# taconite/IntrinsicAvatar

Hardware: AMD Instinct MI355X
Metric: rays/sec (fwd+bwd) at 540×540, 1024 spp; fraction of HBM / MFMA roofline (higher is better)
Workload: dtype f32

## Files before the change

intrinsicavatar_amd/csrc/hashgrid.hip:

```cpp
#include <stdlib.h>

#include "ia_common.h"

namespace {

constexpr int THREADS = 256;
constexpr int MAX_LEVELS = 32;

struct HashCfg {
    int n_levels;
    uint32_t offsets[MAX_LEVELS + 1];
    uint32_t res[MAX_LEVELS];
    float scale[MAX_LEVELS];
};

__host__ void make_cfg(HashCfg& c, int n_levels, int log2_hashmap_size, int base_resolution, float per_level_scale)
{
    c.n_levels = n_levels;
    uint32_t offset = 0;
    const float l2 = log2f(per_level_scale);
    for (int l = 0; l < n_levels; l++) {
        const float sc = exp2f((float)l * l2) * (float)base_resolution - 1.0f;
        const uint32_t res = (uint32_t)ceilf(sc) + 1u;
        const uint32_t max_params = 0xFFFFFFFFu / 2;
        uint32_t p = powf((float)res, 3.0f) > (float)max_params ? max_params : res * res * res;
        p = (p + 7u) / 8u * 8u;
        const uint32_t cap = 1u << log2_hashmap_size;
        if (p > cap) p = cap;
        c.offsets[l] = offset;
        c.res[l] = res;
        c.scale[l] = sc;
        offset += p;
    }
    c.offsets[n_levels] = offset;
}

__device__ __forceinline__ uint32_t grid_index(uint32_t hsize, uint32_t res, uint32_t px, uint32_t py, uint32_t pz)
{
    uint32_t stride = 1, index = 0;
    bool hashed = false;
    index += px * stride; stride *= res;
    if (stride <= hsize) { index += py * stride; stride *= res; } else hashed = true;
    if (!hashed && stride <= hsize) { index += pz * stride; stride *= res; } else hashed = true;
    if (hsize < stride) index = (px * 1u) ^ (py * 2654435761u) ^ (pz * 805459861u);
    return ((hsize & (hsize - 1u)) == 0u) ? (index & (hsize - 1u)) : (index % hsize);
}

typedef float f4_a8 __attribute__((ext_vector_type(4), aligned(8)));

template <bool WITH_JAC>
__global__ __launch_bounds__(THREADS) __attribute__((amdgpu_waves_per_eu(4, 4))) void hash_fwd_kernel(int64_t n, const float* __restrict__ x,
                                                            const float2* __restrict__ params, HashCfg cfg,
                                                            float* __restrict__ out, int out_stride,
                                                            float* __restrict__ dy_dx)
{
    const int L = cfg.n_levels;
    const int64_t t = (int64_t)blockIdx.x * THREADS + threadIdx.x;
    const int64_t i = t / L;
    const int l = (int)(t % L);
    if (i >= n) return;
    const float sc = cfg.scale[l];
    const uint32_t res = cfg.res[l], hsize = cfg.offsets[l + 1] - cfg.offsets[l];
    const float2* tab = params + cfg.offsets[l];
    float pos[3];
    uint32_t pg[3];
#pragma unroll
    for (int d = 0; d < 3; d++) {
        const float p = fmaf(sc, x[i * 3 + d], 0.5f);
        const float fl = floorf(p);
        pg[d] = (uint32_t)(int)fl;
        pos[d] = p - fl;
    }
    float2 v[8];
#pragma unroll
    for (int c = 0; c < 8; c++) {
        const uint32_t idx = grid_index(hsize, res, pg[0] + (c & 1), pg[1] + ((c >> 1) & 1), pg[2] + ((c >> 2) & 1));
        v[c] = tab[idx];
    }
    float a0 = 0.f, a1 = 0.f;
    float j0[3] = {0.f, 0.f, 0.f}, j1[3] = {0.f, 0.f, 0.f};
#pragma unroll
    for (int c = 0; c < 8; c++) {
        const float wx = (c & 1) ? pos[0] : 1.0f - pos[0];
        const float wy = (c & 2) ? pos[1] : 1.0f - pos[1];
        const float wz = (c & 4) ? pos[2] : 1.0f - pos[2];
        const float w = wx * wy * wz;
        a0 = fmaf(w, v[c].x, a0);
        a1 = fmaf(w, v[c].y, a1);
        if (WITH_JAC) {
            const float dx = ((c & 1) ? sc : -sc) * wy * wz;
            const float dy = ((c & 2) ? sc : -sc) * wx * wz;
            const float dz = ((c & 4) ? sc : -sc) * wx * wy;
            j0[0] = fmaf(dx, v[c].x, j0[0]); j0[1] = fmaf(dy, v[c].x, j0[1]); j0[2] = fmaf(dz, v[c].x, j0[2]);
            j1[0] = fmaf(dx, v[c].y, j1[0]); j1[1] = fmaf(dy, v[c].y, j1[1]); j1[2] = fmaf(dz, v[c].y, j1[2]);
        }
    }
    *reinterpret_cast<float2*>(out + i * out_stride + l * 2) = make_float2(a0, a1);
    if (WITH_JAC) {
        float* J = dy_dx + (i * L * 2 + l * 2) * 3;
        J[0] = j0[0]; J[1] = j0[1]; J[2] = j0[2];
        J[3] = j1[0]; J[4] = j1[1]; J[5] = j1[2];
    }
}


struct XcdPlan {
    int first_level[8], n_level[8];
    int part[8], nparts[8];
    int straight;
};

typedef float f4_a8b __attribute__((ext_vector_type(4), aligned(8)));
__device__ __forceinline__ void load_x_pair(const float2* __restrict__ tab, uint32_t i0, uint32_t i1, float2& v0, float2& v1)
{
    if (i1 == i0 + 1u) {
        const f4_a8b q = *reinterpret_cast<const f4_a8b*>(tab + i0);
        v0 = make_float2(q.x, q.y); v1 = make_float2(q.z, q.w);
    } else if (i0 == i1 + 1u) {
        const f4_a8b q = *reinterpret_cast<const f4_a8b*>(tab + i1);
        v1 = make_float2(q.x, q.y); v0 = make_float2(q.z, q.w);
    } else {
        v0 = tab[i0];
        v1 = tab[i1];
    }
}
template <bool WITH_JAC>
__device__ __forceinline__ void xcd_gather(const float2* __restrict__ tab, uint32_t hsize, uint32_t res, float sc,
                                           const float xs[3], float2 v[8], float pos[3])
{
    uint32_t pg[3];
#pragma unroll
    for (int d = 0; d < 3; d++) {
        const float p = fmaf(sc, xs[d], 0.5f);
        const float fl = floorf(p);
        pg[d] = (uint32_t)(int)fl;
        pos[d] = p - fl;
    }
#pragma unroll
    for (int c = 0; c < 8; c += 2) {
        const uint32_t i0 = grid_index(hsize, res, pg[0], pg[1] + ((c >> 1) & 1), pg[2] + ((c >> 2) & 1));
        const uint32_t i1 = grid_index(hsize, res, pg[0] + 1u, pg[1] + ((c >> 1) & 1), pg[2] + ((c >> 2) & 1));
        load_x_pair(tab, i0, i1, v[c], v[c + 1]);
    }
}

template <bool HASHED>
__device__ __forceinline__ uint32_t level_index(uint32_t hsize, uint32_t res, uint32_t px, uint32_t py, uint32_t pz)
{
    if (HASHED) return ((px * 1u) ^ (py * 2654435761u) ^ (pz * 805459861u)) & (hsize - 1u);
    const uint32_t index = px + res * (py + res * pz);
    return min(index >= hsize ? index - hsize : index, hsize - 1u);
}

template <bool HASHED>
__device__ __forceinline__ void xcd_gather2(const float2* __restrict__ tab, uint32_t hsize, uint32_t res, float sc, const float xa[3],
                                            const float xb[3], float2 va[8], float2 vb[8], float pa[3], float pb[3])
{
    typedef float v2f __attribute__((ext_vector_type(2)));
    typedef float f4_a16 __attribute__((ext_vector_type(4), aligned(16)));
    uint32_t ga[3], gb[3];
#pragma unroll
    for (int d = 0; d < 3; d++) {
        const float p = fmaf(sc, xa[d], 0.5f), fl = floorf(p);
        ga[d] = (uint32_t)(int)fl; pa[d] = p - fl;
        const float p2 = fmaf(sc, xb[d], 0.5f), fl2 = floorf(p2);
        gb[d] = (uint32_t)(int)fl2; pb[d] = p2 - fl2;
    }
    uint32_t i0[8], i1[8];
#pragma unroll
    for (int c = 0; c < 4; c++) {
        i0[c] = level_index<HASHED>(hsize, res, ga[0], ga[1] + (c & 1), ga[2] + ((c >> 1) & 1));
        i1[c] = level_index<HASHED>(hsize, res, ga[0] + 1u, ga[1] + (c & 1), ga[2] + ((c >> 1) & 1));
        i0[4 + c] = level_index<HASHED>(hsize, res, gb[0], gb[1] + (c & 1), gb[2] + ((c >> 1) & 1));
        i1[4 + c] = level_index<HASHED>(hsize, res, gb[0] + 1u, gb[1] + (c & 1), gb[2] + ((c >> 1) & 1));
    }
    f4_a16 q[8];
    v2f t[8];
#pragma unroll
    for (int c = 0; c < 8; c++) {
        q[c] = *reinterpret_cast<const f4_a16*>(tab + (i0[c] & ~1u));
        t[c] = *reinterpret_cast<const v2f*>(tab + i1[c]);
    }
#pragma unroll
    for (int c = 0; c < 8; c++) {
        const bool odd = (i0[c] & 1u) != 0u;
        const float2 lo = make_float2(q[c].x, q[c].y), hi = make_float2(q[c].z, q[c].w);
        const float2 e0 = odd ? hi : lo;
        const float2 e1 = (i1[c] == (i0[c] ^ 1u)) ? (odd ? lo : hi) : make_float2(t[c].x, t[c].y);
        if (c < 4) { va[2 * c] = e0; va[2 * c + 1] = e1; } else { vb[2 * (c - 4)] = e0; vb[2 * (c - 4) + 1] = e1; }
    }
    if (!HASHED) {
        if (ga[0] > res || ga[1] > res || ga[2] > res)
#pragma unroll
            for (int c = 0; c < 8; c++) va[c] = tab[grid_index(hsize, res, ga[0] + (c & 1), ga[1] + ((c >> 1) & 1), ga[2] + ((c >> 2) & 1))];
        if (gb[0] > res || gb[1] > res || gb[2] > res)
#pragma unroll
            for (int c = 0; c < 8; c++) vb[c] = tab[grid_index(hsize, res, gb[0] + (c & 1), gb[1] + ((c >> 1) & 1), gb[2] + ((c >> 2) & 1))];
    }
}

template <bool WITH_JAC>
__device__ __forceinline__ void xcd_blend_store(const float2 v[8], const float pos[3], float sc, int64_t slot,
                                                float2* __restrict__ tmp, float* __restrict__ tmp_jac)
{
    float a0 = 0.f, a1 = 0.f;
    float j0[3] = {0.f, 0.f, 0.f}, j1[3] = {0.f, 0.f, 0.f};
#pragma unroll
    for (int c = 0; c < 8; c++) {
        const float wx = (c & 1) ? pos[0] : 1.0f - pos[0];
        const float wy = (c & 2) ? pos[1] : 1.0f - pos[1];
        const float wz = (c & 4) ? pos[2] : 1.0f - pos[2];
        const float w = wx * wy * wz;
        a0 = fmaf(w, v[c].x, a0);
        a1 = fmaf(w, v[c].y, a1);
        if (WITH_JAC) {
            const float dx = ((c & 1) ? sc : -sc) * wy * wz;
            const float dy = ((c & 2) ? sc : -sc) * wx * wz;
            const float dz = ((c & 4) ? sc : -sc) * wx * wy;
            j0[0] = fmaf(dx, v[c].x, j0[0]); j0[1] = fmaf(dy, v[c].x, j0[1]); j0[2] = fmaf(dz, v[c].x, j0[2]);
            j1[0] = fmaf(dx, v[c].y, j1[0]); j1[1] = fmaf(dy, v[c].y, j1[1]); j1[2] = fmaf(dz, v[c].y, j1[2]);
        }
    }
    typedef float v2f __attribute__((ext_vector_type(2)));
    __builtin_nontemporal_store((v2f){a0, a1}, reinterpret_cast<v2f*>(tmp + slot));
    if (WITH_JAC) {
        v2f* J = reinterpret_cast<v2f*>(tmp_jac + slot * 6);
        __builtin_nontemporal_store((v2f){j0[0], j0[1]}, J);
        __builtin_nontemporal_store((v2f){j0[2], j1[0]}, J + 1);
        __builtin_nontemporal_store((v2f){j1[1], j1[2]}, J + 2);
    }
}

template <bool WITH_JAC>
__global__ __launch_bounds__(THREADS) void hash_fwd_xcd_kernel(int64_t n, const float* __restrict__ x,
                                                                const float2* __restrict__ params, HashCfg cfg, XcdPlan plan,
                                                                float2* __restrict__ tmp ,
                                                                float* __restrict__ tmp_jac )
{
    const int slot = blockIdx.x & 7;
    const int64_t chunk = blockIdx.x >> 3, nchunks = gridDim.x >> 3;
    const int np = plan.nparts[slot];
    const int64_t per = (n + np - 1) / np;
    const int64_t lo = per * plan.part[slot], hi = (lo + per < n) ? lo + per : n;
    const int64_t stride = nchunks * THREADS;
    for (int64_t i = lo + chunk * THREADS + threadIdx.x; i < hi; i += 2 * stride) {
        const int64_t i2 = i + stride;
        const bool two = i2 < hi;
        const int64_t ib = two ? i2 : i;
        const float xa[3] = {__builtin_nontemporal_load(x + i * 3 + 0), __builtin_nontemporal_load(x + i * 3 + 1),
                             __builtin_nontemporal_load(x + i * 3 + 2)};
        const float xb[3] = {__builtin_nontemporal_load(x + ib * 3 + 0), __builtin_nontemporal_load(x + ib * 3 + 1),
                             __builtin_nontemporal_load(x + ib * 3 + 2)};
        for (int l = plan.first_level[slot]; l < plan.first_level[slot] + plan.n_level[slot]; l++) {
            const float sc = cfg.scale[l];
            const uint32_t res = cfg.res[l], hsize = cfg.offsets[l + 1] - cfg.offsets[l];
            const float2* tab = params + cfg.offsets[l];
            float2 va[8], vb[8];
            float pa[3], pb[3];
            const uint64_t r64 = res;
            const bool hashed = r64 * r64 * r64 > (uint64_t)hsize;
            if (plan.straight && hashed && (hsize & (hsize - 1u)) == 0u) xcd_gather2<true>(tab, hsize, res, sc, xa, xb, va, vb, pa, pb);
            else if (plan.straight && !hashed) xcd_gather2<false>(tab, hsize, res, sc, xa, xb, va, vb, pa, pb);
            else {
                xcd_gather<WITH_JAC>(tab, hsize, res, sc, xa, va, pa);
                xcd_gather<WITH_JAC>(tab, hsize, res, sc, xb, vb, pb);
            }
            xcd_blend_store<WITH_JAC>(va, pa, sc, (int64_t)l * n + i, tmp, tmp_jac);
            if (two) xcd_blend_store<WITH_JAC>(vb, pb, sc, (int64_t)l * n + i2, tmp, tmp_jac);
        }
    }
}

template <bool WITH_JAC>
__global__ __launch_bounds__(THREADS) void hash_transpose_kernel(int64_t n, int L, const float2* __restrict__ tmp,
                                                                  const float* __restrict__ tmp_jac, float* __restrict__ out,
                                                                  int out_stride, float* __restrict__ dy_dx)
{
    extern __shared__ __attribute__((aligned(16))) float s_t[];
    const int64_t p0 = (int64_t)blockIdx.x * THREADS;
    const int rows = (int)((n - p0) < THREADS ? (n - p0) : THREADS);
    const int ld = 2 * L + 1;
    for (int l = 0; l < L; l++)
        if ((int)threadIdx.x < rows) {
            const float2 v = tmp[(int64_t)l * n + p0 + threadIdx.x];
            s_t[threadIdx.x * ld + 2 * l] = v.x; s_t[threadIdx.x * ld + 2 * l + 1] = v.y;
        }
    __syncthreads();
    for (int i = threadIdx.x; i < rows * 2 * L; i += THREADS) {
        const int r = i / (2 * L), c = i % (2 * L);
        out[(p0 + r) * out_stride + c] = s_t[r * ld + c];
    }
    if (WITH_JAC) {
        __syncthreads();
        const int ldj = 6 * L + 1;
        for (int l = 0; l < L; l++)
            if ((int)threadIdx.x < rows) {
                const float* J = tmp_jac + ((int64_t)l * n + p0 + threadIdx.x) * 6;
#pragma unroll
                for (int k = 0; k < 6; k++) s_t[threadIdx.x * ldj + 6 * l + k] = J[k];
            }
        __syncthreads();
        for (int i = threadIdx.x; i < rows * 6 * L; i += THREADS) {
            const int r = i / (6 * L), c = i % (6 * L);
            dy_dx[(p0 + r) * 6 * L + c] = s_t[r * ldj + c];
        }
    }
}

template <bool SECOND>
__global__ __launch_bounds__(THREADS) void hash_bwd_runs_kernel(int64_t n, const float* __restrict__ x, HashCfg cfg,
                                                                 const float* __restrict__ gE, int gE_stride,
                                                                 const float* __restrict__ gG, int gG_stride,
                                                                 const float* __restrict__ q, float* __restrict__ grad)
{
    const int64_t i = (int64_t)blockIdx.x * THREADS + threadIdx.x;
    const int lane = threadIdx.x & 63;
    const bool active = i < n;
    const int64_t ii = active ? i : n - 1;
    const float x0 = x[ii * 3 + 0], x1 = x[ii * 3 + 1], x2 = x[ii * 3 + 2];
    float qx = 0.f, qy = 0.f, qz = 0.f;
    if (SECOND) { qx = q[ii * 3 + 0]; qy = q[ii * 3 + 1]; qz = q[ii * 3 + 2]; }
    for (int l = 0; l < cfg.n_levels; l++) {
        const float sc = cfg.scale[l];
        const uint32_t res = cfg.res[l], hsize = cfg.offsets[l + 1] - cfg.offsets[l];
        float* tab = grad + (int64_t)cfg.offsets[l] * 2;
        float2 e = make_float2(0.f, 0.f), g = make_float2(0.f, 0.f);
        if (active) {
            if (gE) e = *reinterpret_cast<const float2*>(gE + i * gE_stride + l * 2);
            if (SECOND) g = *reinterpret_cast<const float2*>(gG + i * gG_stride + l * 2);
        }
        const bool any_here = (e.x != 0.f) || (e.y != 0.f) || (g.x != 0.f) || (g.y != 0.f);
        if (!__any(any_here)) continue;
        float pos[3];
        uint32_t pg[3];
        {
            const float xs[3] = {x0, x1, x2};
#pragma unroll
            for (int d = 0; d < 3; d++) {
                const float p = fmaf(sc, xs[d], 0.5f);
                const float fl = floorf(p);
                pg[d] = (uint32_t)(int)fl;
                pos[d] = p - fl;
            }
        }
#pragma unroll
        for (int c = 0; c < 8; c++) {
            const float wx = (c & 1) ? pos[0] : 1.0f - pos[0];
            const float wy = (c & 2) ? pos[1] : 1.0f - pos[1];
            const float wz = (c & 4) ? pos[2] : 1.0f - pos[2];
            const float w0 = wx * wy * wz;
            float vx = e.x * w0, vy = e.y * w0;
            if (SECOND) {
                const float dw = ((c & 1) ? sc : -sc) * wy * wz * qx + ((c & 2) ? sc : -sc) * wx * wz * qy +
                                 ((c & 4) ? sc : -sc) * wx * wy * qz;
                vx += g.x * dw;
                vy += g.y * dw;
            }
            uint32_t idx = grid_index(hsize, res, pg[0] + (c & 1), pg[1] + ((c >> 1) & 1), pg[2] + ((c >> 2) & 1));
            if (!active) { idx = 0xFFFFFFFFu; vx = 0.f; vy = 0.f; }
            const uint32_t prev = __shfl_up(idx, 1, 64);
            const bool head = (lane == 0) || (prev != idx);
            const unsigned long long heads = __ballot(head);
            const unsigned long long below = heads & ((lane == 63) ? ~0ull : ((1ull << (lane + 1)) - 1ull));
            const int hpos = 63 - __clzll(below);
#pragma unroll
            for (int off = 1; off < 64; off <<= 1) {
                const float ax = __shfl_up(vx, off, 64), ay = __shfl_up(vy, off, 64);
                if (lane - off >= hpos) { vx += ax; vy += ay; }
            }
            const bool tail = (lane == 63) || ((heads >> (lane + 1)) & 1ull);
            if (tail && active && (vx != 0.f || vy != 0.f)) {
                unsafeAtomicAdd(tab + (int64_t)idx * 2 + 0, vx);
                unsafeAtomicAdd(tab + (int64_t)idx * 2 + 1, vy);
            }
        }
    }
}


constexpr int SLICE_LOG2 = 13;
constexpr int SLICE = 1 << SLICE_LOG2;
constexpr int BIN_ROUNDS = 4;
constexpr int BIN_TILE = THREADS * BIN_ROUNDS;
constexpr int MAX_BUCKETS = 1024;
constexpr int MAX_PARTS = 64;
constexpr int PART_RECORDS = 1 << 19;

struct BinCfg {
    int n_buckets;
    int bstart[MAX_LEVELS + 1];
};

__host__ void make_bins(BinCfg& b, const HashCfg& c)
{
    int k = 0;
    for (int l = 0; l < c.n_levels; l++) {
        b.bstart[l] = k;
        k += (int)((c.offsets[l + 1] - c.offsets[l] + SLICE - 1) >> SLICE_LOG2);
    }
    b.bstart[c.n_levels] = k;
    b.n_buckets = k;
}

__device__ __forceinline__ void level_max_update(unsigned* p, float lmax)
{
    const unsigned v = __float_as_uint(lmax);
    if (v > __atomic_load_n(p, __ATOMIC_RELAXED)) atomicMax(p, v);
}

template <bool SECOND, bool FILL>
__global__ __launch_bounds__(THREADS) void hash_bin_kernel(int64_t n, const float* __restrict__ x, HashCfg cfg, BinCfg bins,
                                                            const float* __restrict__ gE, int gE_stride,
                                                            const float* __restrict__ gG, int gG_stride,
                                                            const float* __restrict__ q, int nwg,
                                                            int32_t* __restrict__ counts, uint16_t* __restrict__ rec_idx,
                                                            float2* __restrict__ rec_val, uint32_t level_mask,
                                                            unsigned* __restrict__ level_max)
{
    __shared__ int hist[MAX_BUCKETS];
    __shared__ int base[FILL ? MAX_BUCKETS : 1];
    const int lane = threadIdx.x & 63;
// ... 433 lines not shown
}

__global__ __launch_bounds__(THREADS) void sh4_bwd_kernel(int64_t n, const float* __restrict__ d01,
                                                           const float* __restrict__ g, int g_stride,
                                                           float* __restrict__ g_d01)
{
    const int64_t i = (int64_t)blockIdx.x * THREADS + threadIdx.x;
    if (i >= n) return;
    const float x = d01[i * 3 + 0] * 2.f - 1.f, y = d01[i * 3 + 1] * 2.f - 1.f, z = d01[i * 3 + 2] * 2.f - 1.f;
    const float x2 = x * x, y2 = y * y, z2 = z * z;
    const float* go = g + i * g_stride;
    float gx = 0.f, gy = 0.f, gz = 0.f;
    gy += go[1] * -0.48860251190291987f;
    gz += go[2] * 0.48860251190291987f;
    gx += go[3] * -0.48860251190291987f;
    gx += go[4] * 1.0925484305920792f * y;           gy += go[4] * 1.0925484305920792f * x;
    gy += go[5] * -1.0925484305920792f * z;          gz += go[5] * -1.0925484305920792f * y;
    gz += go[6] * 2.0f * 0.94617469575755997f * z;
    gx += go[7] * -1.0925484305920792f * z;          gz += go[7] * -1.0925484305920792f * x;
    gx += go[8] * 2.0f * 0.54627421529603959f * x;   gy += go[8] * -2.0f * 0.54627421529603959f * y;
    gx += go[9] * 0.59004358992664352f * y * (-6.0f * x);
    gy += go[9] * 0.59004358992664352f * (-3.0f * x2 + 3.0f * y2);
    gx += go[10] * 2.8906114426405538f * y * z;      gy += go[10] * 2.8906114426405538f * x * z;
    gz += go[10] * 2.8906114426405538f * x * y;
    gy += go[11] * 0.45704579946446572f * (1.0f - 5.0f * z2);
    gz += go[11] * 0.45704579946446572f * y * (-10.0f * z);
    gz += go[12] * 0.3731763325901154f * (15.0f * z2 - 3.0f);
    gx += go[13] * 0.45704579946446572f * (1.0f - 5.0f * z2);
    gz += go[13] * 0.45704579946446572f * x * (-10.0f * z);
    gx += go[14] * 1.4453057213202769f * z * 2.0f * x; gy += go[14] * 1.4453057213202769f * z * -2.0f * y;
    gz += go[14] * 1.4453057213202769f * (x2 - y2);
    gx += go[15] * 0.59004358992664352f * (-3.0f * x2 + 3.0f * y2);
    gy += go[15] * 0.59004358992664352f * x * 6.0f * y;
    g_d01[i * 3 + 0] = 2.0f * gx; g_d01[i * 3 + 1] = 2.0f * gy; g_d01[i * 3 + 2] = 2.0f * gz;
}

template <int MODE>
__global__ __launch_bounds__(THREADS) void jac_contract_kernel(int64_t n, int K, const float* __restrict__ jac,
                                                                const float* __restrict__ v, int v_stride,
                                                                float* __restrict__ out, int out_stride)
{
    if (MODE == 0) {
        const int64_t i = (int64_t)blockIdx.x * THREADS + threadIdx.x;
        if (i >= n) return;
        float a0 = 0.f, a1 = 0.f, a2 = 0.f;
        const float* J = jac + i * K * 3;
        for (int k = 0; k < K; k++) {
            const float g = v[i * v_stride + k];
            a0 = fmaf(g, J[k * 3 + 0], a0); a1 = fmaf(g, J[k * 3 + 1], a1); a2 = fmaf(g, J[k * 3 + 2], a2);
        }
        out[i * out_stride + 0] = a0; out[i * out_stride + 1] = a1; out[i * out_stride + 2] = a2;
    } else {
        const int64_t t = (int64_t)blockIdx.x * THREADS + threadIdx.x;
        const int64_t i = t / K;
        const int k = (int)(t % K);
        if (i >= n) return;
        const float* J = jac + (i * K + k) * 3;
        out[i * out_stride + k] = J[0] * v[i * v_stride + 0] + J[1] * v[i * v_stride + 1] + J[2] * v[i * v_stride + 2];
    }
}

}

IA_EXPORT int ia_hashgrid_jac_contract(int mode, int64_t n, int K, const float* jac, const float* v, int v_stride,
                                       float* out, int out_stride, ia_stream_t stream)
{
    if (n == 0) return IA_OK;
    IA_REQUIRE(mode == 0 || mode == 1, "mode 0 (J^T v) or 1 (J q)");
    if (mode == 0)
        jac_contract_kernel<0><<<ia::cdiv(n, THREADS), THREADS, 0, (hipStream_t)stream>>>(n, K, jac, v, v_stride, out, out_stride);
    else
        jac_contract_kernel<1><<<ia::cdiv(n * K, THREADS), THREADS, 0, (hipStream_t)stream>>>(n, K, jac, v, v_stride, out, out_stride);
    return ia::check_launch("ia_hashgrid_jac_contract");
}

IA_EXPORT int ia_sh4_bwd(int64_t n, const float* d01, const float* g_sh, int g_stride, float* g_d01, ia_stream_t stream)
{
    if (n == 0) return IA_OK;
    sh4_bwd_kernel<<<ia::cdiv(n, THREADS), THREADS, 0, (hipStream_t)stream>>>(n, d01, g_sh, g_stride, g_d01);
    return ia::check_launch("ia_sh4_bwd");
}

IA_EXPORT int64_t ia_hashgrid_n_entries(int n_levels, int log2_hashmap_size, int base_resolution, float per_level_scale)
{
    if (n_levels <= 0 || n_levels > MAX_LEVELS) return -1;
    HashCfg c;
    make_cfg(c, n_levels, log2_hashmap_size, base_resolution, per_level_scale);
    return (int64_t)c.offsets[n_levels];
}

IA_EXPORT int ia_hashgrid_fwd(int64_t n, const float* x, const float* params, int n_levels, int n_features,
                              int log2_hashmap_size, int base_resolution, float per_level_scale, float* out,
                              int out_stride, float* dy_dx, ia_stream_t stream)
{
    if (n == 0) return IA_OK;
    IA_REQUIRE(n_features == 2, "n_features_per_level must be 2 on this path");
    IA_REQUIRE(n_levels > 0 && n_levels <= MAX_LEVELS, "n_levels out of range");
    IA_REQUIRE(out_stride >= n_levels * 2 && (out_stride % 2) == 0, "out_stride must be even and >= n_levels*2");
    HashCfg c;
    make_cfg(c, n_levels, log2_hashmap_size, base_resolution, per_level_scale);
    const int grid = ia::cdiv(n * n_levels, THREADS);
    hipStream_t s = (hipStream_t)stream;
    if (dy_dx) hash_fwd_kernel<true><<<grid, THREADS, 0, s>>>(n, x, (const float2*)params, c, out, out_stride, dy_dx);
    else hash_fwd_kernel<false><<<grid, THREADS, 0, s>>>(n, x, (const float2*)params, c, out, out_stride, nullptr);
    return ia::check_launch("ia_hashgrid_fwd");
}


struct HashFwdScratch {
    float2* feat;
    float* jac;
    int64_t jac_offset;
};

static size_t hash_fwd_layout(void* scratch, int64_t n, int n_levels, int with_jac, HashFwdScratch* o)
{
    ia::Carver c(nullptr);
    c.take<float2>((size_t)(n * n_levels), 1);
    c.align_to(256);
    o->jac_offset = (int64_t)c.used();
    if (with_jac) c.take<float>((size_t)(n * n_levels) * 6, 1);
    c.skip(256);
    o->feat = reinterpret_cast<float2*>(scratch);
    o->jac = scratch && with_jac ? reinterpret_cast<float*>(reinterpret_cast<char*>(scratch) + o->jac_offset) : nullptr;
    return c.used();
}

IA_EXPORT int64_t ia_hashgrid_fwd_scratch_bytes(int64_t n, int n_levels, int with_jac)
{
    if (n < 0 || n_levels <= 0 || n_levels > MAX_LEVELS) return -1;
    HashFwdScratch w;
    return (int64_t)hash_fwd_layout(nullptr, n, n_levels, with_jac, &w);
}

IA_EXPORT int ia_hashgrid_fwd_xcd(int64_t n, const float* x, const float* params, int n_levels, int n_features,
                                  int log2_hashmap_size, int base_resolution, float per_level_scale, float* out,
                                  int out_stride, float* dy_dx, void* scratch, ia_stream_t stream)
{
    if (n == 0) return IA_OK;
    IA_REQUIRE(n_features == 2, "n_features_per_level must be 2 on this path");
    IA_REQUIRE(n_levels > 0 && n_levels <= MAX_LEVELS, "n_levels out of range");
    IA_REQUIRE((reinterpret_cast<uintptr_t>(params) & 15) == 0, "ia_hashgrid_fwd_xcd: the table must be 16-byte aligned (entry pairs are read with one aligned 16-byte load)");
    IA_REQUIRE(scratch != nullptr, "scratch required");
    HashCfg c;
    make_cfg(c, n_levels, log2_hashmap_size, base_resolution, per_level_scale);
    HashFwdScratch w;
    hash_fwd_layout(scratch, n, n_levels, dy_dx != nullptr, &w);
    float2* tmp = w.feat;
    float* tmp_jac = w.jac;
    const uint32_t cap = 1u << log2_hashmap_size;
    int n_small = 0;
    while (n_small < n_levels && c.offsets[n_small + 1] - c.offsets[n_small] < cap) n_small++;
    hipStream_t s = (hipStream_t)stream;
    static int chunks_jac = 0, chunks_plain = 0;
    if (!chunks_plain) {
        int dev = 0, n_cu = 256, b0 = 0, b1 = 0;
        (void)hipGetDevice(&dev);
        (void)hipDeviceGetAttribute(&n_cu, hipDeviceAttributeMultiprocessorCount, dev);
        (void)hipOccupancyMaxActiveBlocksPerMultiprocessor(&b0, hash_fwd_xcd_kernel<false>, THREADS, 0);
        (void)hipOccupancyMaxActiveBlocksPerMultiprocessor(&b1, hash_fwd_xcd_kernel<true>, THREADS, 0);
        (void)hipGetLastError();
        const int per_xcd = n_cu >= 8 ? n_cu / 8 : 1;
        chunks_plain = (b0 > 6 ? 6 : (b0 > 0 ? b0 : 4)) * per_xcd;
        chunks_jac = (b1 > 6 ? 6 : (b1 > 0 ? b1 : 4)) * per_xcd;
        if (const char* e = getenv("IA_HASH_XCD_CHUNKS")) chunks_plain = chunks_jac = atoi(e);
    }
    const int chunks = dy_dx ? chunks_jac : chunks_plain;
    int l = n_small;
    bool small_done = (n_small == 0);
    static const int plan_env = getenv("IA_HASH_XCD_PLAN") ? (getenv("IA_HASH_XCD_PLAN")[0] == 'p' ? 1 : 2) : 0;
    const bool by_level = plan_env == 2 || (plan_env == 0 && n >= 300000);
    static const int lpl = getenv("IA_HASH_LEVELS_PER_LAUNCH") ? max(1, atoi(getenv("IA_HASH_LEVELS_PER_LAUNCH"))) : 1;
    if (by_level) {
        for (int u = (n_small > 0 ? -1 : 0); u < n_levels - n_small; u += (u < 0 ? 1 : lpl)) {
            XcdPlan plan;
            plan.straight = 1;
            for (int k = 0; k < 8; k++) {
                plan.first_level[k] = u < 0 ? 0 : n_small + u;
                plan.n_level[k] = u < 0 ? n_small : min(lpl, n_levels - n_small - u);
                plan.part[k] = k; plan.nparts[k] = 8;
            }
            if (dy_dx) hash_fwd_xcd_kernel<true><<<8 * chunks, THREADS, 0, s>>>(n, x, (const float2*)params, c, plan, tmp, tmp_jac);
            else hash_fwd_xcd_kernel<false><<<8 * chunks, THREADS, 0, s>>>(n, x, (const float2*)params, c, plan, tmp, nullptr);
        }
        l = n_levels;
        small_done = true;
    }
    while (l < n_levels || !small_done) {
        XcdPlan plan;
        plan.straight = 1;
        const int big_left = n_levels - l;
        if (big_left >= 8) {
            for (int k = 0; k < 8; k++) { plan.first_level[k] = l + k; plan.n_level[k] = 1; plan.part[k] = 0; plan.nparts[k] = 1; }
            l += 8;
        } else {
            const int units = big_left + (small_done ? 0 : 1);
            static const float small_cost = getenv("IA_HASH_SMALL_COST") ? (float)atof(getenv("IA_HASH_SMALL_COST")) : 1.0f;
            float w[9];
            int share[9], used = 0;
            for (int u = 0; u < units; u++) { w[u] = (!small_done && u == units - 1) ? small_cost : 1.0f; share[u] = 1; used++; }
            for (; used < 8; used++) {
                int best = 0;
                for (int u = 1; u < units; u++) if (w[u] / share[u] > w[best] / share[best]) best = u;
                share[best]++;
            }
            int k = 0;
            for (int u = 0; u < units; u++) {
                const bool is_small = (!small_done && u == units - 1);
                for (int j = 0; j < share[u]; j++, k++) {
                    plan.first_level[k] = is_small ? 0 : l + u;
                    plan.n_level[k] = is_small ? n_small : 1;
                    plan.part[k] = j; plan.nparts[k] = share[u];
                }
            }
            l = n_levels;
            small_done = true;
        }
        if (dy_dx) hash_fwd_xcd_kernel<true><<<8 * chunks, THREADS, 0, s>>>(n, x, (const float2*)params, c, plan, tmp, tmp_jac);
        else hash_fwd_xcd_kernel<false><<<8 * chunks, THREADS, 0, s>>>(n, x, (const float2*)params, c, plan, tmp, nullptr);
    }
    if (out == nullptr) return ia::check_launch("ia_hashgrid_fwd_xcd");
    const size_t lds = sizeof(float) * THREADS * (dy_dx ? 6 * n_levels + 1 : 2 * n_levels + 1);
    static bool attr = false;
    if (!attr) {
        (void)hipFuncSetAttribute((const void*)hash_transpose_kernel<true>, hipFuncAttributeMaxDynamicSharedMemorySize, 128 * 1024);
        (void)hipGetLastError();
        attr = true;
    }
    if (dy_dx) hash_transpose_kernel<true><<<ia::cdiv(n, THREADS), THREADS, lds, s>>>(n, n_levels, tmp, tmp_jac, out, out_stride, dy_dx);
    else hash_transpose_kernel<false><<<ia::cdiv(n, THREADS), THREADS, lds, s>>>(n, n_levels, tmp, nullptr, out, out_stride, nullptr);
    return ia::check_launch("ia_hashgrid_fwd_xcd");
}

IA_EXPORT int64_t ia_hashgrid_fwd_levels_jac_offset(int64_t n, int n_levels)
{
    HashFwdScratch w;
    hash_fwd_layout(nullptr, n, n_levels, 1, &w);
    return w.jac_offset;
}

IA_EXPORT int ia_hashgrid_fwd_levels(int64_t n, const float* x, const float* params, int n_levels, int n_features, int log2_hashmap_size,
                                     int base_resolution, float per_level_scale, int with_jac, void* scratch, ia_stream_t stream)
{
    return ia_hashgrid_fwd_xcd(n, x, params, n_levels, n_features, log2_hashmap_size, base_resolution, per_level_scale, nullptr, 0,
                               with_jac ? reinterpret_cast<float*>(scratch) : nullptr, scratch, stream);
}

IA_EXPORT int ia_hashgrid_bwd(int64_t n, const float* x, int n_levels, int n_features, int log2_hashmap_size,
                              int base_resolution, float per_level_scale, const float* g_enc, int g_enc_stride,
                              const float* g_jac, int g_jac_stride, const float* q, float* grad_params,
                              ia_stream_t stream)
{
    if (n == 0) return IA_OK;
    IA_REQUIRE(n_features == 2, "n_features_per_level must be 2 on this path");
    IA_REQUIRE(n_levels > 0 && n_levels <= MAX_LEVELS, "n_levels out of range");
    IA_REQUIRE(g_enc != nullptr || g_jac != nullptr, "need g_enc and/or g_jac");
    IA_REQUIRE((g_jac == nullptr) == (q == nullptr), "g_jac and q go together");
    HashCfg c;
    make_cfg(c, n_levels, log2_hashmap_size, base_resolution, per_level_scale);
    hipStream_t s = (hipStream_t)stream;
    const int grid = ia::cdiv(n, THREADS);
    if (g_jac) hash_bwd_runs_kernel<true><<<grid, THREADS, 0, s>>>(n, x, c, g_enc, g_enc_stride, g_jac, g_jac_stride, q, grad_params);
    else hash_bwd_runs_kernel<false><<<grid, THREADS, 0, s>>>(n, x, c, g_enc, g_enc_stride, nullptr, 0, nullptr, grad_params);
    return ia::check_launch("ia_hashgrid_bwd");
}


namespace {
struct BinLayout {
    int nwg; int64_t m, records;
    int32_t *counts, *total;
    unsigned* level_max;
    int32_t* plan;
    void* tmp;
    float2* rec_val;
    uint16_t* rec_idx;
    bool fits;
};
bool staged_fill()
{
    static int mode = -1;
    if (mode < 0) {
        const char* e = getenv("IA_HASHBWD_FILL");
        mode = (e && e[0] == 'd') ? 0 : 1;
    }
    return mode == 1;
}

size_t bin_layout(void* scratch, size_t bytes, int64_t n, int n_levels, int n_buckets, BinLayout* L)
{
    L->nwg = staged_fill() ? ia::cdiv(n, U_PTS) : ia::cdiv(n, BIN_TILE);
    L->m = (int64_t)n_buckets * L->nwg;
    L->records = n * n_levels * 8;
    ia::Carver c(scratch, bytes);
    L->counts = c.take<int32_t>((size_t)L->m);
    L->total = c.take<int32_t>(1);
    L->level_max = c.take<unsigned>(MAX_LEVELS);
    L->plan = c.take<int32_t>(MAX_BUCKETS + 64);
    L->tmp = c.take<char>((size_t)ia_scan_tmp_bytes(L->m));
    L->rec_val = c.take<float2>((size_t)L->records);
    L->rec_idx = c.take<uint16_t>((size_t)L->records);
    L->fits = c.fits();
    return c.need(1);
}
}

IA_EXPORT int64_t ia_hashgrid_bwd_scratch_bytes(int64_t n, int n_levels, int log2_hashmap_size, int base_resolution,
                                                float per_level_scale)
{
    if (n_levels <= 0 || n_levels > MAX_LEVELS || n < 0) return -1;
    HashCfg c;
    make_cfg(c, n_levels, log2_hashmap_size, base_resolution, per_level_scale);
    BinCfg b;
    make_bins(b, c);
    if (b.n_buckets > MAX_BUCKETS) return -1;
    BinLayout L;
    return (int64_t)bin_layout(nullptr, SIZE_MAX, n, n_levels, b.n_buckets, &L);
}

IA_EXPORT int ia_hashgrid_bwd_binned(int64_t n, const float* x, int n_levels, int n_features, int log2_hashmap_size,
                                     int base_resolution, float per_level_scale, const float* g_enc, int g_enc_stride,
                                     const float* g_jac, int g_jac_stride, const float* q, float* grad_params,
                                     uint32_t level_mask, void* scratch, int64_t scratch_bytes, ia_stream_t stream)
{
    if (n == 0) return IA_OK;
    IA_REQUIRE(n_features == 2, "n_features_per_level must be 2 on this path");
    IA_REQUIRE(n_levels > 0 && n_levels <= MAX_LEVELS, "n_levels out of range");
    IA_REQUIRE(g_enc != nullptr || g_jac != nullptr, "need g_enc and/or g_jac");
    IA_REQUIRE((g_jac == nullptr) == (q == nullptr), "g_jac and q go together");
    IA_REQUIRE(n * n_levels * 8 < (int64_t)0x7FFFFFFF, "n too large for 32-bit record offsets: split the batch");
    HashCfg c;
    make_cfg(c, n_levels, log2_hashmap_size, base_resolution, per_level_scale);
    BinCfg b;
    make_bins(b, c);
    IA_REQUIRE(b.n_buckets <= MAX_BUCKETS, "too many (level, slice) buckets");
    BinLayout L;
    bin_layout(scratch, scratch_bytes > 0 ? (size_t)scratch_bytes : 0, n, n_levels, b.n_buckets, &L);
    IA_REQUIRE(scratch != nullptr && L.fits, "scratch smaller than ia_hashgrid_bwd_scratch_bytes(n)");
    int32_t *counts = L.counts, *total = L.total;
    void* tmp = L.tmp;
    float2* rec_val = L.rec_val;
    uint16_t* rec_idx = L.rec_idx;
    hipStream_t s = (hipStream_t)stream;
    unsigned* level_max = L.level_max;
    if (hipMemsetAsync(level_max, 0, MAX_LEVELS * sizeof(unsigned), s) != hipSuccess) return ia::check_launch("ia_hashgrid_bwd_binned(memset)");
    const bool staged = staged_fill();
    const int ugrid = ia::cdiv(L.nwg, U_WAVES);
    constexpr size_t lds_count = (size_t)U_WAVES * MAX_BUCKETS * sizeof(int), lds_fill = (size_t)U_WAVES * sizeof(UnitLds);
    if (staged) {
        if (g_jac) hash_bin_unit_kernel<true, false><<<ugrid, THREADS, lds_count, s>>>(n, x, c, b, g_enc, g_enc_stride, g_jac, g_jac_stride, q, L.nwg, L.m, counts, total, rec_idx, rec_val, level_mask, level_max);
        else hash_bin_unit_kernel<false, false><<<ugrid, THREADS, lds_count, s>>>(n, x, c, b, g_enc, g_enc_stride, nullptr, 0, nullptr, L.nwg, L.m, counts, total, rec_idx, rec_val, level_mask, level_max);
    } else {
        if (g_jac) hash_bin_kernel<true, false><<<L.nwg, THREADS, 0, s>>>(n, x, c, b, g_enc, g_enc_stride, g_jac, g_jac_stride, q, L.nwg, counts, rec_idx, rec_val, level_mask, level_max);
        else hash_bin_kernel<false, false><<<L.nwg, THREADS, 0, s>>>(n, x, c, b, g_enc, g_enc_stride, nullptr, 0, nullptr, L.nwg, counts, rec_idx, rec_val, level_mask, level_max);
    }
    int r = ia_exclusive_scan_i32(counts, counts, total, L.m, tmp, stream);
    if (r != IA_OK) return r;
    static bool attr_fill = false;
    if (staged && !attr_fill) {
        (void)hipFuncSetAttribute((const void*)hash_bin_unit_kernel<true, true>, hipFuncAttributeMaxDynamicSharedMemorySize, (int)lds_fill);
        (void)hipFuncSetAttribute((const void*)hash_bin_unit_kernel<false, true>, hipFuncAttributeMaxDynamicSharedMemorySize, (int)lds_fill);
        (void)hipGetLastError();
        attr_fill = true;
    }
    if (staged) {
        if (g_jac) hash_bin_unit_kernel<true, true><<<ugrid, THREADS, lds_fill, s>>>(n, x, c, b, g_enc, g_enc_stride, g_jac, g_jac_stride, q, L.nwg, L.m, counts, total, rec_idx, rec_val, level_mask, level_max);
        else hash_bin_unit_kernel<false, true><<<ugrid, THREADS, lds_fill, s>>>(n, x, c, b, g_enc, g_enc_stride, nullptr, 0, nullptr, L.nwg, L.m, counts, total, rec_idx, rec_val, level_mask, level_max);
    } else {
        if (g_jac) hash_bin_kernel<true, true><<<L.nwg, THREADS, 0, s>>>(n, x, c, b, g_enc, g_enc_stride, g_jac, g_jac_stride, q, L.nwg, counts, rec_idx, rec_val, level_mask, level_max);
        else hash_bin_kernel<false, true><<<L.nwg, THREADS, 0, s>>>(n, x, c, b, g_enc, g_enc_stride, nullptr, 0, nullptr, L.nwg, counts, rec_idx, rec_val, level_mask, level_max);
    }
    static bool attr = false;
// ... 20 lines not shown
```

Baseline: 1.008 million.

## Generalize hashgrid XCD gather to N points per thread with single-entry loads

The XCD forward kernel now processes a compile-time number of points per thread (4 without Jacobian, 2 with) instead of a fixed two, to put more independent gathers in flight and hide hash-table latency. It also adds a load mode that fetches each corner as a separate 8-byte load instead of a 16-byte pair load plus a fallback, and makes that the default. Occupancy-based chunk sizing is now computed per kernel variant. More points per thread raises register pressure and may lower occupancy.

```diff
diff --git a/intrinsicavatar_amd/csrc/hashgrid.hip b/intrinsicavatar_amd/csrc/hashgrid.hip
--- a/intrinsicavatar_amd/csrc/hashgrid.hip
+++ b/intrinsicavatar_amd/csrc/hashgrid.hip
@@ -1,4 +1,5 @@
 #include <stdlib.h>
+#include <string.h>
 
 #include "ia_common.h"
 
@@ -152,50 +153,70 @@
     return min(index >= hsize ? index - hsize : index, hsize - 1u);
 }
 
-template <bool HASHED>
-__device__ __forceinline__ void xcd_gather2(const float2* __restrict__ tab, uint32_t hsize, uint32_t res, float sc, const float xa[3],
-                                            const float xb[3], float2 va[8], float2 vb[8], float pa[3], float pb[3])
+enum { HASH_LOADS_PAIR = 0, HASH_LOADS_SINGLE = 1 };
+#ifndef IA_HASH_NPTS
+#define IA_HASH_NPTS 4
+#endif
+#ifndef IA_HASH_NPTS_JAC
+#define IA_HASH_NPTS_JAC 2
+#endif
+
+template <bool HASHED, int LOADS, int NPTS>
+__device__ __forceinline__ void xcd_gather2(const float2* __restrict__ tab, uint32_t hsize, uint32_t res, float sc,
+                                            const float (&xs)[NPTS][3], float2 (&v)[NPTS][8], float (&pos)[NPTS][3])
 {
     typedef float v2f __attribute__((ext_vector_type(2)));
     typedef float f4_a16 __attribute__((ext_vector_type(4), aligned(16)));
-    uint32_t ga[3], gb[3];
-#pragma unroll
-    for (int d = 0; d < 3; d++) {
-        const float p = fmaf(sc, xa[d], 0.5f), fl = floorf(p);
-        ga[d] = (uint32_t)(int)fl; pa[d] = p - fl;
-        const float p2 = fmaf(sc, xb[d], 0.5f), fl2 = floorf(p2);
-        gb[d] = (uint32_t)(int)fl2; pb[d] = p2 - fl2;
-    }
-    uint32_t i0[8], i1[8];
-#pragma unroll
-    for (int c = 0; c < 4; c++) {
-        i0[c] = level_index<HASHED>(hsize, res, ga[0], ga[1] + (c & 1), ga[2] + ((c >> 1) & 1));
-        i1[c] = level_index<HASHED>(hsize, res, ga[0] + 1u, ga[1] + (c & 1), ga[2] + ((c >> 1) & 1));
-        i0[4 + c] = level_index<HASHED>(hsize, res, gb[0], gb[1] + (c & 1), gb[2] + ((c >> 1) & 1));
-        i1[4 + c] = level_index<HASHED>(hsize, res, gb[0] + 1u, gb[1] + (c & 1), gb[2] + ((c >> 1) & 1));
-    }
-    f4_a16 q[8];
-    v2f t[8];
-#pragma unroll
-    for (int c = 0; c < 8; c++) {
-        q[c] = *reinterpret_cast<const f4_a16*>(tab + (i0[c] & ~1u));
-        t[c] = *reinterpret_cast<const v2f*>(tab + i1[c]);
-    }
-#pragma unroll
-    for (int c = 0; c < 8; c++) {
-        const bool odd = (i0[c] & 1u) != 0u;
-        const float2 lo = make_float2(q[c].x, q[c].y), hi = make_float2(q[c].z, q[c].w);
-        const float2 e0 = odd ? hi : lo;
-        const float2 e1 = (i1[c] == (i0[c] ^ 1u)) ? (odd ? lo : hi) : make_float2(t[c].x, t[c].y);
-        if (c < 4) { va[2 * c] = e0; va[2 * c + 1] = e1; } else { vb[2 * (c - 4)] = e0; vb[2 * (c - 4) + 1] = e1; }
+    uint32_t g[NPTS][3];
+#pragma unroll
+    for (int d = 0; d < 3; d++)
+#pragma unroll
+        for (int p = 0; p < NPTS; p++) {
+            const float q = fmaf(sc, xs[p][d], 0.5f), fl = floorf(q);
+            g[p][d] = (uint32_t)(int)fl; pos[p][d] = q - fl;
+        }
+    uint32_t i0[4 * NPTS], i1[4 * NPTS];
+#pragma unroll
+    for (int c = 0; c < 4; c++)
+#pragma unroll
+        for (int p = 0; p < NPTS; p++) {
+            i0[4 * p + c] = level_index<HASHED>(hsize, res, g[p][0], g[p][1] + (c & 1), g[p][2] + ((c >> 1) & 1));
+            i1[4 * p + c] = level_index<HASHED>(hsize, res, g[p][0] + 1u, g[p][1] + (c & 1), g[p][2] + ((c >> 1) & 1));
+        }
+    if (LOADS == HASH_LOADS_SINGLE) {
+        v2f e0[4 * NPTS], e1[4 * NPTS];
+#pragma unroll
+        for (int c = 0; c < 4 * NPTS; c++) {
+            e0[c] = *reinterpret_cast<const v2f*>(tab + i0[c]);
+            e1[c] = *reinterpret_cast<const v2f*>(tab + i1[c]);
+        }
+#pragma unroll
+        for (int c = 0; c < 4 * NPTS; c++) {
+            v[c >> 2][2 * (c & 3)] = make_float2(e0[c].x, e0[c].y);
+            v[c >> 2][2 * (c & 3) + 1] = make_float2(e1[c].x, e1[c].y);
+        }
+    } else {
+        f4_a16 q[4 * NPTS];
+        v2f t[4 * NPTS];
+#pragma unroll
+        for (int c = 0; c < 4 * NPTS; c++) {
+            q[c] = *reinterpret_cast<const f4_a16*>(tab + (i0[c] & ~1u));
+            t[c] = *reinterpret_cast<const v2f*>(tab + i1[c]);
+        }
+#pragma unroll
+        for (int c = 0; c < 4 * NPTS; c++) {
+            const bool odd = (i0[c] & 1u) != 0u;
+            const float2 lo = make_float2(q[c].x, q[c].y), hi = make_float2(q[c].z, q[c].w);
+            v[c >> 2][2 * (c & 3)] = odd ? hi : lo;
+            v[c >> 2][2 * (c & 3) + 1] = (i1[c] == (i0[c] ^ 1u)) ? (odd ? lo : hi) : make_float2(t[c].x, t[c].y);
+        }
     }
     if (!HASHED) {
-        if (ga[0] > res || ga[1] > res || ga[2] > res)
-#pragma unroll
-            for (int c = 0; c < 8; c++) va[c] = tab[grid_index(hsize, res, ga[0] + (c & 1), ga[1] + ((c >> 1) & 1), ga[2] + ((c >> 2) & 1))];
-        if (gb[0] > res || gb[1] > res || gb[2] > res)
-#pragma unroll
-            for (int c = 0; c < 8; c++) vb[c] = tab[grid_index(hsize, res, gb[0] + (c & 1), gb[1] + ((c >> 1) & 1), gb[2] + ((c >> 2) & 1))];
+#pragma unroll
+        for (int p = 0; p < NPTS; p++)
+            if (g[p][0] > res || g[p][1] > res || g[p][2] > res)
+#pragma unroll
+                for (int c = 0; c < 8; c++) v[p][c] = tab[grid_index(hsize, res, g[p][0] + (c & 1), g[p][1] + ((c >> 1) & 1), g[p][2] + ((c >> 2) & 1))];
     }
 }
 
@@ -231,7 +252,7 @@
     }
 }
 
-template <bool WITH_JAC>
+template <bool WITH_JAC, int LOADS, int NPTS>
 __global__ __launch_bounds__(THREADS) void hash_fwd_xcd_kernel(int64_t n, const float* __restrict__ x,
                                                                 const float2* __restrict__ params, HashCfg cfg, XcdPlan plan,
                                                                 float2* __restrict__ tmp ,
@@ -243,30 +264,33 @@
     const int64_t per = (n + np - 1) / np;
     const int64_t lo = per * plan.part[slot], hi = (lo + per < n) ? lo + per : n;
     const int64_t stride = nchunks * THREADS;
-    for (int64_t i = lo + chunk * THREADS + threadIdx.x; i < hi; i += 2 * stride) {
-        const int64_t i2 = i + stride;
-        const bool two = i2 < hi;
-        const int64_t ib = two ? i2 : i;
-        const float xa[3] = {__builtin_nontemporal_load(x + i * 3 + 0), __builtin_nontemporal_load(x + i * 3 + 1),
-                             __builtin_nontemporal_load(x + i * 3 + 2)};
-        const float xb[3] = {__builtin_nontemporal_load(x + ib * 3 + 0), __builtin_nontemporal_load(x + ib * 3 + 1),
-                             __builtin_nontemporal_load(x + ib * 3 + 2)};
+    for (int64_t i = lo + chunk * THREADS + threadIdx.x; i < hi; i += NPTS * stride) {
+        bool on[NPTS];
+        float xs[NPTS][3];
+#pragma unroll
+        for (int p = 0; p < NPTS; p++) {
+            on[p] = i + p * stride < hi;
+            const int64_t ip = on[p] ? i + p * stride : i;
+#pragma unroll
+            for (int d = 0; d < 3; d++) xs[p][d] = __builtin_nontemporal_load(x + ip * 3 + d);
+        }
         for (int l = plan.first_level[slot]; l < plan.first_level[slot] + plan.n_level[slot]; l++) {
             const float sc = cfg.scale[l];
             const uint32_t res = cfg.res[l], hsize = cfg.offsets[l + 1] - cfg.offsets[l];
             const float2* tab = params + cfg.offsets[l];
-            float2 va[8], vb[8];
-            float pa[3], pb[3];
+            float2 v[NPTS][8];
+            float pos[NPTS][3];
             const uint64_t r64 = res;
             const bool hashed = r64 * r64 * r64 > (uint64_t)hsize;
-            if (plan.straight && hashed && (hsize & (hsize - 1u)) == 0u) xcd_gather2<true>(tab, hsize, res, sc, xa, xb, va, vb, pa, pb);
-            else if (plan.straight && !hashed) xcd_gather2<false>(tab, hsize, res, sc, xa, xb, va, vb, pa, pb);
+            if (plan.straight && hashed && (hsize & (hsize - 1u)) == 0u) xcd_gather2<true, LOADS, NPTS>(tab, hsize, res, sc, xs, v, pos);
+            else if (plan.straight && !hashed) xcd_gather2<false, LOADS, NPTS>(tab, hsize, res, sc, xs, v, pos);
             else {
-                xcd_gather<WITH_JAC>(tab, hsize, res, sc, xa, va, pa);
-                xcd_gather<WITH_JAC>(tab, hsize, res, sc, xb, vb, pb);
-            }
-            xcd_blend_store<WITH_JAC>(va, pa, sc, (int64_t)l * n + i, tmp, tmp_jac);
-            if (two) xcd_blend_store<WITH_JAC>(vb, pb, sc, (int64_t)l * n + i2, tmp, tmp_jac);
+#pragma unroll
+                for (int p = 0; p < NPTS; p++) xcd_gather<WITH_JAC>(tab, hsize, res, sc, xs[p], v[p], pos[p]);
+            }
+#pragma unroll
+            for (int p = 0; p < NPTS; p++)
+                if (on[p]) xcd_blend_store<WITH_JAC>(v[p], pos[p], sc, (int64_t)l * n + i + p * stride, tmp, tmp_jac);
         }
     }
 }
@@ -1006,20 +1030,29 @@
     int n_small = 0;
     while (n_small < n_levels && c.offsets[n_small + 1] - c.offsets[n_small] < cap) n_small++;
     hipStream_t s = (hipStream_t)stream;
-    static int chunks_jac = 0, chunks_plain = 0;
-    if (!chunks_plain) {
-        int dev = 0, n_cu = 256, b0 = 0, b1 = 0;
+    typedef void (*xcd_kernel_t)(int64_t, const float*, const float2*, HashCfg, XcdPlan, float2*, float*);
+    static const xcd_kernel_t kernels[2][2] = {
+        {hash_fwd_xcd_kernel<false, HASH_LOADS_PAIR, IA_HASH_NPTS>, hash_fwd_xcd_kernel<false, HASH_LOADS_SINGLE, IA_HASH_NPTS>},
+        {hash_fwd_xcd_kernel<true, HASH_LOADS_PAIR, IA_HASH_NPTS_JAC>, hash_fwd_xcd_kernel<true, HASH_LOADS_SINGLE, IA_HASH_NPTS_JAC>}};
+    const int jac = dy_dx ? 1 : 0;
+    int loads = HASH_LOADS_SINGLE;
+    if (const char* e = getenv("IA_HASH_LOADS")) {
+        IA_REQUIRE(!strcmp(e, "pair") || !strcmp(e, "single"), "IA_HASH_LOADS must be pair or single");
+        loads = e[0] == 's' ? HASH_LOADS_SINGLE : HASH_LOADS_PAIR;
+    }
+    const xcd_kernel_t kernel = kernels[jac][loads];
+    static int chunks_of[2][2] = {{0, 0}, {0, 0}};
+    if (!chunks_of[jac][loads]) {
+        int dev = 0, n_cu = 256, b0 = 0;
         (void)hipGetDevice(&dev);
         (void)hipDeviceGetAttribute(&n_cu, hipDeviceAttributeMultiprocessorCount, dev);
-        (void)hipOccupancyMaxActiveBlocksPerMultiprocessor(&b0, hash_fwd_xcd_kernel<false>, THREADS, 0);
-        (void)hipOccupancyMaxActiveBlocksPerMultiprocessor(&b1, hash_fwd_xcd_kernel<true>, THREADS, 0);
+        (void)hipOccupancyMaxActiveBlocksPerMultiprocessor(&b0, kernel, THREADS, 0);
         (void)hipGetLastError();
         const int per_xcd = n_cu >= 8 ? n_cu / 8 : 1;
-        chunks_plain = (b0 > 6 ? 6 : (b0 > 0 ? b0 : 4)) * per_xcd;
-        chunks_jac = (b1 > 6 ? 6 : (b1 > 0 ? b1 : 4)) * per_xcd;
-        if (const char* e = getenv("IA_HASH_XCD_CHUNKS")) chunks_plain = chunks_jac = atoi(e);
-    }
-    const int chunks = dy_dx ? chunks_jac : chunks_plain;
+        chunks_of[jac][loads] = (b0 > 6 ? 6 : (b0 > 0 ? b0 : 4)) * per_xcd;
+    }
+    int chunks = chunks_of[jac][loads];
+    if (const char* e = getenv("IA_HASH_XCD_CHUNKS")) chunks = max(1, atoi(e));
     int l = n_small;
     bool small_done = (n_small == 0);
     static const int plan_env = getenv("IA_HASH_XCD_PLAN") ? (getenv("IA_HASH_XCD_PLAN")[0] == 'p' ? 1 : 2) : 0;
@@ -1034,8 +1067,7 @@
                 plan.n_level[k] = u < 0 ? n_small : min(lpl, n_levels - n_small - u);
                 plan.part[k] = k; plan.nparts[k] = 8;
             }
-            if (dy_dx) hash_fwd_xcd_kernel<true><<<8 * chunks, THREADS, 0, s>>>(n, x, (const float2*)params, c, plan, tmp, tmp_jac);
-            else hash_fwd_xcd_kernel<false><<<8 * chunks, THREADS, 0, s>>>(n, x, (const float2*)params, c, plan, tmp, nullptr);
+            kernel<<<8 * chunks, THREADS, 0, s>>>(n, x, (const float2*)params, c, plan, tmp, tmp_jac);
         }
         l = n_levels;
         small_done = true;
@@ -1070,8 +1102,7 @@
             l = n_levels;
             small_done = true;
         }
-        if (dy_dx) hash_fwd_xcd_kernel<true><<<8 * chunks, THREADS, 0, s>>>(n, x, (const float2*)params, c, plan, tmp, tmp_jac);
-        else hash_fwd_xcd_kernel<false><<<8 * chunks, THREADS, 0, s>>>(n, x, (const float2*)params, c, plan, tmp, nullptr);
+        kernel<<<8 * chunks, THREADS, 0, s>>>(n, x, (const float2*)params, c, plan, tmp, tmp_jac);
     }
     if (out == nullptr) return ia::check_launch("ia_hashgrid_fwd_xcd");
     const size_t lds = sizeof(float) * THREADS * (dy_dx ? 6 * n_levels + 1 : 2 * n_levels + 1);
```

New measurement: 1.012 million (median of 6 runs). Within noise of the previous version (+0.4%).
